# JosephCatrambone/aruco3

Measured on AMD Instinct MI355X. Metric: frames/sec at 1920x1080 ARUCO dict, higher is better.
Workload: dtype u8

## Files before the change

### aruco3_amd/csrc/k_contours.hip

```cpp
#include <algorithm>
#include <cmath>

#include "a3_common.h"
#include "a3_launch.h"


namespace a3 {

constexpr int kFinB = 8;
constexpr int kScatB = 1;

struct Nb8 { uint64_t c; uint64_t n[8]; };

__device__ __forceinline__ uint64_t ldw(const uint64_t* __restrict__ img, int wpr, int H, int j, int y) {
    return (y >= 0 && y < H && j >= 0 && j < wpr) ? img[(size_t)y * wpr + j] : 0ull;
}

__device__ __forceinline__ void pdart_words(const Nb8& nb, uint64_t p[8]) {
#pragma unroll
    for (int k = 0; k < 8; k++) {
        uint64_t m = nb.c & nb.n[k] & ~nb.n[(k + 7) & 7];
        if ((k & 1) == 0) m &= ~nb.n[(k + 6) & 7];
        p[k] = m;
    }
// ... 1055 lines not shown

__global__ __launch_bounds__(256) void k_resolve_eval(const FinState* __restrict__ fin, uint32_t n_darts, int W,
                                                      const uint64_t* __restrict__ d_rec, const uint64_t* __restrict__ t_cur,
                                                      uint64_t* __restrict__ t_next, int iter, DeviceCounters* __restrict__ ctr,
                                                      const uint32_t* __restrict__ n_live) {
    if (!ctr->resolve_needed || (iter > 0 && ctr->resolve_changed[iter - 1] == 0)) return;
    if (n_live) n_darts = min(n_darts, *n_live);
    for (uint32_t d = blockIdx.x * blockDim.x + threadIdx.x; d < n_darts; d += gridDim.x * blockDim.x) {
        const uint64_t rec = d_rec[d];
        const uint32_t info = rec_info(rec);
        if (!(info & (kInfoW | kInfoE))) continue;
        const uint32_t my_leader = fin[d].leader;
        if (fin[my_leader].leader != my_leader) { atomicOr(&ctr->err_flags, kErrBrokenEvent); continue; }
        const uint32_t xy = rec_xy(rec);
        const uint32_t x = xy & 0xFFFF, y = xy >> 16;
        const uint32_t q = y * (uint32_t)W + x;
        const uint32_t F = rec_F(rec), P = pdart_mask(F);
        const int k = info & 7;
        const uint32_t base = d - __popc(P & ((1u << k) - 1u));
        const int cnt = __popc(P);
        bool wfires = true;
        for (int i = 0; i < cnt; i++) {
            const uint32_t leader = fin[base + i].leader;
            const uint32_t t = (uint32_t)(t_cur[leader] >> 32);
            if (t < 2u * q) { wfires = false; break; }
        }
        const bool has_w = x > 0 && !(F & 1u);
        uint32_t key = kNoKey;
        if ((info & kInfoW) && wfires) key = 2u * q;
        else if ((info & kInfoE) && !(has_w && wfires)) key = 2u * q + 1u;
        if (key != kNoKey) atomicMin(reinterpret_cast<unsigned long long*>(&t_next[my_leader]),
                                     (unsigned long long)(((uint64_t)key << 32) | d));
    }
}

__global__ void k_resolve_commit(const FinState* __restrict__ fin, uint32_t n_darts, uint64_t* __restrict__ t_cur,
                                 uint64_t* __restrict__ t_next, int iter, int last, DeviceCounters* __restrict__ ctr,
                                 const uint32_t* __restrict__ n_live) {
    if (!ctr->resolve_needed || (iter > 0 && ctr->resolve_changed[iter - 1] == 0)) return;
    if (n_live) n_darts = min(n_darts, *n_live);
    uint32_t changed = 0;
    for (uint32_t d = blockIdx.x * blockDim.x + threadIdx.x; d < n_darts; d += gridDim.x * blockDim.x) {
        if (fin[d].leader != d) continue;
        const uint64_t a = t_cur[d], b = t_next[d];
        if (a != b) { changed++; t_cur[d] = b; }
        t_next[d] = kInf64;
    }
    for (int o = 32; o > 0; o >>= 1) changed += __shfl_down(changed, o);
    if ((threadIdx.x & 63) == 0 && changed) {
        atomicAdd(&ctr->resolve_changed[iter], changed);
        if (last) atomicOr(&ctr->err_flags, kErrResolve);
    }
}

__global__ __launch_bounds__(256) void k_cycle_select(FinState* fin, const uint32_t* __restrict__ leader_list,
                                                      const unsigned int* __restrict__ leader_count, const uint32_t* __restrict__ d_succ,
                                                      const uint64_t* __restrict__ t_cur, const uint32_t* __restrict__ frame_base,
                                                      uint32_t n_frames, uint32_t first_frame, uint32_t min_edge_length, double eps_factor,
                                                      double image_diag, ContourRec* __restrict__ contours,
                                                      uint32_t* __restrict__ cyc_start_off, uint32_t max_contours, uint64_t max_points,
                                                      DeviceCounters* __restrict__ ctr, uint32_t shard_cap, const uint64_t* __restrict__ d_rec,
                                                      int W ,
                                                      uint32_t* __restrict__ keep_tmp ,
                                                      int keep_all ,
                                                      const EntryState* __restrict__ es ) {
    if (ctr->entry_overflow) return;
    __shared__ uint32_t s_wave[4], s_wave_t[4];
    __shared__ unsigned long long s_wave_p[4];
    __shared__ uint32_t s_cbase;
    __shared__ unsigned long long s_pbase;
    const int lane = threadIdx.x & 63, wave = threadIdx.x >> 6;
    uint32_t n_max = 0;
    for (uint32_t sh = 0; sh < kLeaderShards; sh++) n_max = max(n_max, leader_count[sh]);
    const uint32_t span = (n_max + 63u) & ~63u;
    const uint32_t n_leaders = span * kLeaderShards;
    const uint32_t stride = gridDim.x * blockDim.x;

    struct Eval { bool valid, traced, keep, broken; uint32_t n, d; uint64_t t; };
    auto eval = [&](uint32_t i0) -> Eval {
        Eval e{false, false, false, false, 0u, 0u, kInf64};
        const uint32_t sh = i0 / span, i = i0 - sh * span;
        e.valid = i < leader_count[sh];
        if (!e.valid) return e;
        e.d = leader_list[(size_t)sh * shard_cap + i];
        e.t = W > 0 ? dart_key(e.d, d_rec[e.d], W) : t_cur[e.d];
        e.traced = e.t != kInf64;
        if (!e.traced) return e;
        const uint32_t sl = d_succ[e.d];
        const FinState fsl = fin_final(fin[sl], sl, es);
        if (sl == e.d || fsl.leader != e.d) { e.broken = true; return e; }
        e.n = (fsl.w & kFinHops) + 1u;
        const double eps = (double)e.n * eps_factor;
        e.keep = keep_all || (e.n >= 5u && (uint64_t)e.n * e.n >= 8ull * min_edge_length && eps < image_diag + 1.0);
        return e;
    };

    uint32_t my_keep = 0, my_traced = 0;
    unsigned long long my_points = 0;
    bool broken = false, moved = false;
    for (uint32_t i0 = blockIdx.x * blockDim.x + threadIdx.x; i0 < n_leaders; i0 += stride) {
        const Eval e = eval(i0);
        my_traced += e.traced; my_keep += e.keep; my_points += e.keep ? e.n : 0u;
        broken |= e.broken;
        if (e.valid) { const uint32_t sh = i0 / span; keep_tmp[(size_t)sh * shard_cap + (i0 - sh * span)] = e.keep ? 1u : 0u; }
        if (W > 0 && e.valid && !natural_start_fires(e.d, fin, es, d_rec, W)) moved = true;
    }
    if (moved) ctr->resolve_needed = 1u;
    if (broken) atomicOr(&ctr->err_flags, kErrBrokenEvent);
    uint32_t inc_k = my_keep, inc_t = my_traced;
    unsigned long long inc_p = my_points;
#define A3_DPP_ADD64(V, CTRL, RM)                                                                                       \
    {                                                                                                                    \
        const uint32_t lo_ = (uint32_t)__builtin_amdgcn_update_dpp(0, (int)(uint32_t)(V), CTRL, RM, 0xF, false);           \
        const uint32_t hi_ = (uint32_t)__builtin_amdgcn_update_dpp(0, (int)(uint32_t)((V) >> 32), CTRL, RM, 0xF, false);    \
        (V) += ((unsigned long long)hi_ << 32) | lo_;                                                                    \
    }
#define A3_DPP_ADD32(V, CTRL, RM) (V) += (uint32_t)__builtin_amdgcn_update_dpp(0, (int)(V), CTRL, RM, 0xF, false);
#define A3_STEP(CTRL, RM) A3_DPP_ADD32(inc_k, CTRL, RM) A3_DPP_ADD32(inc_t, CTRL, RM) A3_DPP_ADD64(inc_p, CTRL, RM)
    A3_STEP(0x111, 0xF) A3_STEP(0x112, 0xF) A3_STEP(0x114, 0xF) A3_STEP(0x118, 0xF) A3_STEP(0x142, 0xA) A3_STEP(0x143, 0xC)
#undef A3_STEP
#undef A3_DPP_ADD32
#undef A3_DPP_ADD64
    if (lane == 63) { s_wave[wave] = inc_k; s_wave_p[wave] = inc_p; s_wave_t[wave] = inc_t; }
    __syncthreads();
    uint32_t base_k = 0, tot_k = 0;
    unsigned long long base_p = 0, tot_p = 0;
    for (int w = 0; w < 4; w++) {
        if (w < wave) { base_k += s_wave[w]; base_p += s_wave_p[w]; }
        tot_k += s_wave[w]; tot_p += s_wave_p[w];
    }
    if (threadIdx.x == 0) {
        const uint32_t tot_t = s_wave_t[0] + s_wave_t[1] + s_wave_t[2] + s_wave_t[3];
        if (tot_t) atomicAdd(&ctr->traced, tot_t);
        s_cbase = tot_k ? atomicAdd(&ctr->contours, tot_k) : 0u;
        s_pbase = tot_k ? atomicAdd(&ctr->points, tot_p) : 0ull;
    }
    __syncthreads();
    uint32_t c = s_cbase + base_k + (inc_k - my_keep);
    unsigned long long pb = s_pbase + base_p + (inc_p - my_points);

    for (uint32_t i0 = blockIdx.x * blockDim.x + threadIdx.x; i0 < n_leaders; i0 += stride) {
        {
            const uint32_t sh = i0 / span, i = i0 - sh * span;
            if (i >= leader_count[sh]) continue;
            if (!keep_tmp[(size_t)sh * shard_cap + i]) { const uint32_t d = leader_list[(size_t)sh * shard_cap + i]; fin[d] = FinState{d, kFinEvent | kFinHops}; continue; }
        }
        const Eval e = eval(i0);
        if (!e.valid) continue;
        uint32_t slot = kNone;
        if (e.keep) {
            if (c >= max_contours || c >= kFinHops) atomicOr(&ctr->err_flags, kErrContourTable);
            else if (pb + e.n > max_points) atomicOr(&ctr->err_flags, kErrPointPool);
            else {
                uint32_t lo = 0, hi = n_frames;
                while (hi - lo > 1) { const uint32_t mid = (lo + hi) >> 1; if (frame_base[mid] <= e.d) lo = mid; else hi = mid; }
                ContourRec r;
                r.frame = first_frame + lo;
                r.start_key = (uint32_t)(e.t >> 32);
                r.point_base = (uint32_t)pb;
                r.n = e.n;
                contours[c] = r;
                cyc_start_off[c] = (uint32_t)e.t == e.d ? 0u : fin_final(fin[(uint32_t)e.t], (uint32_t)e.t, es).w & kFinHops;
                slot = c;
            }
            c++; pb += e.n;
        }
        fin[e.d] = FinState{e.d, kFinEvent | (slot == kNone ? kFinHops : slot)};
    }
}

__global__ __launch_bounds__(256) void k_scatter_points(const FinState* __restrict__ fin, uint32_t n_darts, const uint64_t* __restrict__ d_rec,
                                                        const ContourRec* __restrict__ contours,
                                                        const uint32_t* __restrict__ cyc_start_off, uint32_t* __restrict__ points,
                                                        const uint32_t* __restrict__ n_live, DeviceCounters* __restrict__ ctr,
                                                        uint32_t max_contours, uint64_t max_points,
                                                        const EntryState* __restrict__ es ) {
    if (ctr->entry_overflow) return;
    if (n_live) n_darts = min(n_darts, *n_live);
    const uint32_t n_contours = min(ctr->contours, max_contours);
    bool bad = false;
    constexpr int B = kScatB;
    const uint32_t stride = gridDim.x * blockDim.x;
    for (uint32_t d0 = blockIdx.x * blockDim.x + threadIdx.x; d0 < n_darts; d0 += B * stride) {
        FinState s[B];
        uint64_t rec[B];
        uint32_t c[B], so[B];
        FinState ls[B];
        ContourRec r[B];
        bool live[B];
#pragma unroll
        for (int u = 0; u < B; u++) {
            const uint32_t d = min(d0 + (uint32_t)u * stride, n_darts - 1u);
            s[u] = fin_final(fin[d], d, es);
        }
#pragma unroll
        for (int u = 0; u < B; u++) {
            live[u] = d0 + (uint32_t)u * stride < n_darts && (s[u].w & kFinEvent) != 0u &&
                      (s[u].w & kFinDead) == 0u;
            const uint32_t leader = live[u] ? s[u].leader : 0u;
            ls[u] = fin[leader];
            c[u] = ls[u].w & kFinHops;
            rec[u] = live[u] ? d_rec[min(d0 + (uint32_t)u * stride, n_darts - 1u)] : 0ull;
        }
#pragma unroll
        for (int u = 0; u < B; u++) {
            const bool named = live[u] && ls[u].leader == s[u].leader && c[u] != kFinHops;
            live[u] = named && c[u] < n_contours;
            bad |= named && !live[u];
            r[u] = contours[live[u] ? c[u] : 0u];
            so[u] = cyc_start_off[live[u] ? c[u] : 0u];
        }
#pragma unroll
        for (int u = 0; u < B; u++) {
            if (!live[u]) continue;
            const uint32_t off = s[u].leader == d0 + (uint32_t)u * stride ? 0u : s[u].w & kFinHops;
            const uint32_t rank = so[u] >= off ? so[u] - off : so[u] + r[u].n - off;
            if (rank < r[u].n && (uint64_t)r[u].point_base + rank < max_points) points[r[u].point_base + rank] = rec_xy(rec[u]);
            else bad = true;
        }
    }
    if (bad) atomicOr(&ctr->err_flags, kErrScatter);
}

__device__ __forceinline__ int orient(int px, int py, int qx, int qy, int rx, int ry) {
    const long long v = (long long)(qy - py) * (rx - qx) - (long long)(qx - px) * (ry - qy);
    return v == 0 ? 0 : (v > 0 ? 1 : -1);
}

__device__ bool hull4(const int* __restrict__ in , int* __restrict__ out ) {
    int sp = 0;
    for (int i = 1; i < 4; i++)
        if (in[2 * i + 1] < in[2 * sp + 1] || (in[2 * i + 1] == in[2 * sp + 1] && in[2 * i] < in[2 * sp])) sp = i;
    const int sx = in[2 * sp], sy = in[2 * sp + 1];
    int qx[3], qy[3];
    {
        int tx[4], ty[4];
        for (int i = 0; i < 4; i++) { tx[i] = in[2 * i]; ty[i] = in[2 * i + 1]; }
        tx[sp] = tx[0]; ty[sp] = ty[0];
        for (int i = 0; i < 3; i++) { qx[i] = tx[i + 1]; qy[i] = ty[i + 1]; }
    }
    for (int i = 1; i < 3; i++) {
        const int ax = qx[i], ay = qy[i];
        int j = i;
        while (j > 0) {
            const int bx = qx[j - 1], by = qy[j - 1];
            const int o = orient(sx, sy, ax, ay, bx, by);
            bool less;
            if (o == 0) {
                const long long da = (long long)(ax - sx) * (ax - sx) + (long long)(ay - sy) * (ay - sy);
                const long long db = (long long)(bx - sx) * (bx - sx) + (long long)(by - sy) * (by - sy);
                less = da < db;
            } else less = (o == -1);
            if (!less) break;
            qx[j] = bx; qy[j] = by; j--;
        }
        qx[j] = ax; qy[j] = ay;
    }
    int hx[5], hy[5], sn = 1;
    hx[0] = sx; hy[0] = sy;
    for (int i = 0; i < 3; i++) {
        while (sn > 1 && orient(hx[sn - 2], hy[sn - 2], hx[sn - 1], hy[sn - 1], qx[i], qy[i]) != -1) sn--;
        hx[sn] = qx[i]; hy[sn] = qy[i]; sn++;
    }
    if (sn != 4) return false;
    for (int i = 0; i < 4; i++) { out[2 * i] = hx[i]; out[2 * i + 1] = hy[i]; }
    return true;
}

__device__ __forceinline__ void enforce_clockwise(int* __restrict__ hq ) {
    const int dx1 = hq[2] - hq[0], dy1 = hq[3] - hq[1], dx2 = hq[4] - hq[0], dy2 = hq[5] - hq[1];
    if (dx1 * dy2 - dy1 * dx2 < 0) { const int tx = hq[2], ty = hq[3]; hq[2] = hq[6]; hq[3] = hq[7]; hq[6] = tx; hq[7] = ty; }
}

__global__ void k_debug_clockwise(const int32_t* __restrict__ in, uint32_t n, int32_t* __restrict__ out) {
    const uint32_t i = blockIdx.x * blockDim.x + threadIdx.x;
    if (i >= n) return;
    int q[8];
    for (int k = 0; k < 8; k++) q[k] = in[8 * i + k];
    enforce_clockwise(q);
    for (int k = 0; k < 8; k++) out[8 * i + k] = q[k];
}

#define A3_DPP_MAX64(V, CTRL, ROWMASK)                                                                                   \
    {                                                                                                                    \
        const uint32_t lo_ = (uint32_t)__builtin_amdgcn_update_dpp(0, (int)(uint32_t)(V), CTRL, ROWMASK, 0xF, false);        \
        const uint32_t hi_ = (uint32_t)__builtin_amdgcn_update_dpp(0, (int)(uint32_t)((V) >> 32), CTRL, ROWMASK, 0xF, false); \
        const unsigned long long o_ = ((unsigned long long)hi_ << 32) | lo_;                                             \
        (V) = o_ > (V) ? o_ : (V);                                                                                       \
    }
template <int G>
__device__ __forceinline__ unsigned long long group_max_u64(unsigned long long v) {
    A3_DPP_MAX64(v, 0x111, 0xF)
    A3_DPP_MAX64(v, 0x112, 0xF)
    A3_DPP_MAX64(v, 0x114, 0xF)
    A3_DPP_MAX64(v, 0x118, 0xF)
    if constexpr (G == 16) return __shfl(v, 15, 16);
    A3_DPP_MAX64(v, 0x142, 0xA)
    A3_DPP_MAX64(v, 0x143, 0xC)
    const uint32_t lo = (uint32_t)__builtin_amdgcn_readlane((int)(uint32_t)v, 63), hi = (uint32_t)__builtin_amdgcn_readlane((int)(uint32_t)(v >> 32), 63);
    return ((unsigned long long)hi << 32) | lo;
}
#undef A3_DPP_MAX64

constexpr uint32_t kSmallBorder = 64;
template <int G>
__device__ __forceinline__ void contour_quads_body(uint32_t block, uint32_t n_blocks, const ContourRec* __restrict__ contours, const DeviceCounters* __restrict__ ctr,
                                                       uint32_t max_contours, const uint32_t* __restrict__ points, double eps_factor,
                                                       uint32_t min_edge_length, uint32_t first_frame, uint32_t max_cand,
                                                       CandRec* __restrict__ cands, uint32_t* __restrict__ cand_count,
                                                       unsigned int* __restrict__ err_flags, bool coords14) {
    if (ctr->err_flags & (kErrPointPool | kErrContourTable)) return;
    const uint32_t n_contours = min(ctr->contours, max_contours);
    const int lane = threadIdx.x & (G - 1);
    const uint32_t wave_global = (block * blockDim.x + threadIdx.x) / G, n_waves = (n_blocks * blockDim.x) / G;
    for (uint32_t c = wave_global; c < n_contours; c += n_waves) {
        const ContourRec r = contours[c];
        if ((r.n <= kSmallBorder) != (G == 16)) continue;
        const uint32_t* P = points + r.point_base;
        const uint32_t n = r.n;
        const double eps = (double)n * eps_factor;
        uint32_t seg_a[8], seg_b[8];
        int nseg = 1, splits = 0;
        uint32_t kept[3];
        seg_a[0] = 0; seg_b[0] = n - 1;
        bool reject = false;
        while (nseg > 0 && !reject) {
            nseg--;
            const uint32_t a = seg_a[nseg], b = seg_b[nseg];
            const uint32_t pa = P[a], pb = P[b];
            const int ax = pa & 0xFFFF, ay = pa >> 16, bx = pb & 0xFFFF, by = pb >> 16;
            const int la = ay - by, lb = bx - ax;
            const long long lc = (long long)ax * by - (long long)bx * ay;
            unsigned long long best = 0;
            for (uint32_t i0 = a + 1 + lane; i0 <= b; i0 += 4 * G) {
                uint32_t p[4];
#pragma unroll
                for (int u = 0; u < 4; u++) p[u] = P[min(i0 + (uint32_t)u * G, b)];
#pragma unroll
                for (int u = 0; u < 4; u++) {
                    const uint32_t i = i0 + (uint32_t)u * G;
                    if (i > b) break;
                    unsigned long long anum;
                    if (coords14) {
                        const int v = __mul24(la, (int)(p[u] & 0xFFFF)) + __mul24(lb, (int)(p[u] >> 16)) + (int)lc;
                        anum = (unsigned long long)(uint32_t)(v < 0 ? -v : v);
                    } else {
                        long long num = (long long)la * (int)(p[u] & 0xFFFF) + (long long)lb * (int)(p[u] >> 16) + lc;
                        anum = (unsigned long long)(num < 0 ? -num : num);
                    }
                    const unsigned long long cand = (anum << 30) | (unsigned long long)(~i & 0x3FFFFFFFu);
                    if (cand > best) best = cand;
                }
            }
            best = group_max_u64<G>(best);
            const unsigned long long num = best >> 30;
            if (num == 0) continue;
            const uint32_t index = ~(uint32_t)best & 0x3FFFFFFFu;
            const double dn = (double)num, den = (double)((long long)la * la + (long long)lb * lb);
            const double lhs = dn * dn, rhs = eps * eps * den;
            bool far;
            if (lhs > rhs * (1.0 + 1e-9)) far = true;
            else if (lhs < rhs * (1.0 - 1e-9)) far = false;
            else far = dn / sqrt(den) > eps;
            if (far) {
                if (splits == 3) { reject = true; break; }
                kept[splits++] = index;
                seg_a[nseg] = a; seg_b[nseg] = index; nseg++;
                seg_a[nseg] = index; seg_b[nseg] = b; nseg++;
            }
        }
        if (reject || splits != 3) continue;
        if (lane != 0) continue;
        uint32_t k0 = kept[0], k1 = kept[1], k2 = kept[2], t;
        if (k0 > k1) { t = k0; k0 = k1; k1 = t; }
        if (k1 > k2) { t = k1; k1 = k2; k2 = t; }
        if (k0 > k1) { t = k0; k0 = k1; k1 = t; }
        const uint32_t idx[4] = {0u, k0, k1, k2};
        int q[8], hq[8];
        for (int i = 0; i < 4; i++) { const uint32_t p = P[idx[i]]; q[2 * i] = p & 0xFFFF; q[2 * i + 1] = p >> 16; }
        if (!hull4(q, hq)) continue;
        uint32_t cmin = min_edge_length + 1u;
        for (int i = 0; i < 4; i++) {
            const int j = (i + 1) & 3;
            const int dx = hq[2 * i] - hq[2 * j], dy = hq[2 * i + 1] - hq[2 * j + 1];
            const uint32_t d2 = (uint32_t)(dx * dx + dy * dy);
            cmin = d2 < cmin ? d2 : cmin;
        }
        if (cmin < min_edge_length) continue;
        enforce_clockwise(hq);
        const uint32_t fl = r.frame - first_frame;
        const uint32_t slot = atomicAdd(&cand_count[fl], 1u);
        if (slot >= max_cand) { atomicOr(err_flags, kErrCandTable); continue; }
        CandRec cr;
        cr.start_key = r.start_key;
        for (int i = 0; i < 8; i++) cr.xy[i] = (uint16_t)hq[i];
        cands[(size_t)fl * max_cand + slot] = cr;
    }
}

__global__ __launch_bounds__(256) void k_contour_quads(uint32_t blocks64, const ContourRec* __restrict__ contours, const DeviceCounters* __restrict__ ctr,
                                                       uint32_t max_contours, const uint32_t* __restrict__ points, double eps_factor,
                                                       uint32_t min_edge_length, uint32_t first_frame, uint32_t max_cand,
                                                       CandRec* __restrict__ cands, uint32_t* __restrict__ cand_count,
                                                       unsigned int* __restrict__ err_flags, int coords14) {
    if (blockIdx.x < blocks64)
        contour_quads_body<64>(blockIdx.x, blocks64, contours, ctr, max_contours, points, eps_factor, min_edge_length, first_frame, max_cand, cands,
                               cand_count, err_flags, coords14 != 0);
    else
        contour_quads_body<16>(blockIdx.x - blocks64, gridDim.x - blocks64, contours, ctr, max_contours, points, eps_factor, min_edge_length,
                               first_frame, max_cand, cands, cand_count, err_flags, coords14 != 0);
}

__global__ void k_unpack_bits(const uint64_t* __restrict__ bits, int W, int H, uint8_t* __restrict__ out) {
    const int x = blockIdx.x * blockDim.x + threadIdx.x, y = blockIdx.y;
    if (x >= W) return;
    const int wpr = (int)words_per_row((uint32_t)W);
    out[(size_t)y * W + x] = ((bits[(size_t)y * wpr + (x >> 6)] >> (x & 63)) & 1ull) ? 255 : 0;
}

constexpr int kFinBlocks = 1536;
static inline int blocks_for(uint64_t n, int per_block, int cap) {
    uint64_t b = (n + per_block - 1) / per_block;
    if (b < 1) b = 1;
    if (b > (uint64_t)cap) b = cap;
    return (int)b;
}

__global__ __launch_bounds__(256) void k_zero(uint4* __restrict__ p, uint32_t n16) {
    for (uint32_t i = blockIdx.x * blockDim.x + threadIdx.x; i < n16; i += gridDim.x * blockDim.x) p[i] = make_uint4(0u, 0u, 0u, 0u);
}
hipError_t launch_zero(hipStream_t st, void* p, size_t bytes) {
    const uint32_t n16 = (uint32_t)(bytes / 16);
    hipLaunchKernelGGL(k_zero, dim3(blocks_for(n16, 256, 256)), dim3(256), 0, st, reinterpret_cast<uint4*>(p), n16);
    return hipGetLastError();
}

static size_t tile_off_offset(uint32_t W, uint32_t H, uint32_t n_frames) { return (size_t)dart_tiles(W, H) * n_frames; }
static size_t tile_mask_offset_bytes(uint32_t W, uint32_t H, uint32_t n_frames) { return ((size_t)dart_tiles(W, H) * n_frames * 4 * (1 + kCountHalves) + 7) & ~(size_t)7; }
size_t tile_darts_bytes(uint32_t W, uint32_t H, uint32_t n_frames) { return tile_mask_offset_bytes(W, H, n_frames) + (size_t)dart_tiles(W, H) * n_frames * kCountHalves * 8; }

hipError_t launch_dart_count(hipStream_t st, const DartCountLaunch& d) {
    const uint64_t* const bits = d.bits; const int W = d.W, H = d.H; const uint32_t first_frame = d.first_frame, n_frames = d.n_frames;
    unsigned long long* const frame_darts = d.frame_darts; uint32_t* const tile_darts = d.tile_darts; PlanWords* const plan = d.plan;
    const uint32_t tiles_x = dart_tiles_x((uint32_t)W), tiles_y = ((uint32_t)H + kTileRows - 1) / kTileRows;
    const uint32_t wpr = words_per_row((uint32_t)W);
    uint32_t* h1 = tile_darts + (size_t)tiles_x * tiles_y * n_frames * 2;
    unsigned long long* tmask = reinterpret_cast<unsigned long long*>(reinterpret_cast<uint8_t*>(tile_darts) + tile_mask_offset_bytes((uint32_t)W, (uint32_t)H, n_frames));
    if (wpr <= 30)
        hipLaunchKernelGGL(k_dart_count<32>, dim3((tiles_y + 1) / 2, n_frames, kCountHalves), dim3(64), 0, st, bits, W, H, first_frame, frame_darts, tile_darts, h1, tmask);
    else
        hipLaunchKernelGGL(k_dart_count<64>, dim3(((wpr + kCountLanes - 1) / kCountLanes) * tiles_y, n_frames, kCountHalves), dim3(64), 0, st, bits, W, H, first_frame,
                           frame_darts, tile_darts, h1, tmask);
    hipLaunchKernelGGL(k_tile_scan, dim3(n_frames + (plan ? 1u : 0u)), dim3(256), 0, st, tile_darts, h1, tiles_x * tiles_y, first_frame,
                       tile_darts + (size_t)tiles_x * tiles_y * n_frames, n_frames, frame_darts, (unsigned long long)d.plan_cap, d.frame_base, plan,
                       reinterpret_cast<uint4*>(d.zero_p), (uint32_t)(d.zero_bytes / 16));
    return hipGetLastError();
}

hipError_t launch_dart_build(hipStream_t st, const ContourChunk& c) {
    const uint32_t tiles = dart_tiles((uint32_t)c.W, (uint32_t)c.H);
    const uint32_t* const tile_off = c.tile_darts + tile_off_offset((uint32_t)c.W, (uint32_t)c.H, c.batch_frames);
    const unsigned long long* const tile_mask = reinterpret_cast<const unsigned long long*>(
        reinterpret_cast<const uint8_t*>(c.tile_darts) + tile_mask_offset_bytes((uint32_t)c.W, (uint32_t)c.H, c.batch_frames));
    hipLaunchKernelGGL(k_dart_assign, dim3((tiles * c.n_frames + 7u) / 8u * 8u), dim3(256), 0, st, c.bits, c.W, c.H, c.first_frame, c.frame_base, tile_off,
                       c.pix_base, c.tile_darts, c.d_rec, c.d_succ, c.n_live, c.dbg, tile_mask, tiles, c.n_frames);
    if (c.dbg && c.dbg != 5) return hipGetLastError();
    hipLaunchKernelGGL(k_dart_link, dim3(blocks_for(c.n_darts, 256, 4096)), dim3(256), 0, st, c.W, c.H, c.first_frame, c.pix_base, c.bits, c.d_rec, c.d_succ,
                       c.n_darts, c.n_live);
    return hipGetLastError();
}

size_t entry_state_bytes() { return sizeof(EntryState); }
static bool finalize_inline(bool frame_entries, bool trust_natural) { return frame_entries && trust_natural; }
size_t fin_state_bytes() { return sizeof(FinState); }
size_t entry_slots(uint32_t n_darts) { return (size_t)entry_shard_cap(n_darts) * kEntryShards; }
size_t leader_list_bytes(uint32_t n_darts) { return (size_t)leader_shard_cap(n_darts) * kLeaderShards * 4; }

hipError_t launch_rank_cycles(hipStream_t st, const ContourChunk& c) {
    const uint32_t n_darts = c.n_darts, n_frames = c.n_frames, min_edge_length = c.min_edge_length; const int W = c.W, dbg = c.dbg, phase = c.phase;
    const uint64_t* const d_rec = c.d_rec; const uint32_t* const d_succ = c.d_succ, * const n_live = c.n_live, * const frame_base = c.frame_base;
    uint32_t* const entry_list = c.entry_list, * const leader_list = c.leader_list, * const frame_entries = c.frame_entries;
    unsigned int* const entry_count = c.entry_count, * const leader_count = c.leader_count, * const dead_count = c.dead_count;
    DeviceCounters* const ctr = c.ctr;
    const int trust_natural = c.inline_resolve_W > 0 ? 1 : 0;
    const uint32_t ecap = entry_shard_cap(n_darts);
    FinState* fin = reinterpret_cast<FinState*>(c.fin);
    const bool no_finalize = finalize_inline(frame_entries != nullptr, trust_natural != 0) && dbg == 0;
    uint32_t* const ll = no_finalize ? leader_list : nullptr;
    const uint32_t lcap = leader_shard_cap(n_darts);
    if (phase != 2) {
        if (frame_entries && !dead_count)
            hipLaunchKernelGGL((k_local_contract<kLTFrame, false>), dim3((n_darts + kLTFrame - 1) / kLTFrame), dim3(256), 0, st, n_darts, W, d_rec, d_succ, fin,
                               entry_list, entry_count, ecap, frame_base, frame_entries, n_live, dbg, min_edge_length, dead_count, trust_natural,
                               ll, leader_count, lcap);
        else if (frame_entries)
            hipLaunchKernelGGL((k_local_contract<kLTFrame, true>), dim3((n_darts + kLTFrame - 1) / kLTFrame), dim3(256), 0, st, n_darts, W, d_rec, d_succ, fin,
                               entry_list, entry_count, ecap, frame_base, frame_entries, n_live, dbg, min_edge_length, dead_count, trust_natural,
                               ll, leader_count, lcap);
        else
            hipLaunchKernelGGL((k_local_contract<kLT, true>), dim3((n_darts + kLT - 1) / kLT), dim3(256), 0, st, n_darts, W, d_rec, d_succ, fin,
                               entry_list, entry_count, ecap, frame_base, frame_entries, n_live, dbg, min_edge_length, dead_count, trust_natural,
                               ll, leader_count, lcap);
    }
    if (dbg || phase == 1) return hipGetLastError();
    EntryState* a = reinterpret_cast<EntryState*>(c.es_a);
    EntryState* b = reinterpret_cast<EntryState*>(c.es_b);
    if (frame_entries) {
        hipLaunchKernelGGL(k_entry_frame, dim3(n_frames), dim3(256), 0, st, entry_list, frame_entries, frame_base, fin, d_rec, W, a, ctr,
                           ll, leader_count, lcap);
        if (no_finalize) return hipGetLastError();
        const int fin_blocks = std::max(blocks_for(n_darts, 256, kFinBlocks), (int)(((uint64_t)n_darts + 256ull * 32 - 1) / (256ull * 32)));
        hipLaunchKernelGGL(k_jump_finalize, dim3(fin_blocks), dim3(256), 0, st, n_darts, a, fin,
                           leader_list, leader_count, leader_shard_cap(n_darts), n_live, ctr);
        return hipGetLastError();
    }
    const dim3 grid(blocks_for(n_darts / 16 + 1, 256, 1024)), block(256);
    hipLaunchKernelGGL(k_entry_init, grid, block, 0, st, entry_list, entry_count, fin, d_rec, W, a, ecap);
    for (int r = 0; r < c.max_rounds; r++) {
        hipLaunchKernelGGL(k_entry_jump, grid, block, 0, st, a, b, entry_count, ecap, r, ctr);
        EntryState* t = a; a = b; b = t;
    }
    const int fin_blocks = std::max(blocks_for(n_darts, 256, kFinBlocks), (int)(((uint64_t)n_darts + 256ull * 32 - 1) / (256ull * 32)));
    hipLaunchKernelGGL(k_jump_finalize, dim3(fin_blocks), block, 0, st, n_darts, a, fin,
                       leader_list, leader_count, leader_shard_cap(n_darts), n_live, ctr);
    return hipGetLastError();
}

hipError_t launch_resolve(hipStream_t st, const ContourChunk& c) {
    const uint32_t n_darts = c.n_darts; const int W = c.W, max_iters = c.resolve_iters;
    const uint64_t* const d_rec = c.d_rec; uint64_t* const t_cur = c.t_cur, * const t_next = c.t_next;
    const uint32_t* const leader_list = c.leader_list, * const n_live = c.n_live; const unsigned int* const leader_count = c.leader_count;
    DeviceCounters* const ctr = c.ctr;
    const FinState* fin = reinterpret_cast<const FinState*>(c.fin);
    if (max_iters <= 0) return hipSuccess;
    const dim3 grid(blocks_for(n_darts, 256, 4096)), block(256);
    hipLaunchKernelGGL(k_resolve_fast, dim3(blocks_for(n_darts / 16 + 1, 256, 1024)), block, 0, st, fin, leader_list, leader_count,
                       leader_shard_cap(n_darts), W, d_rec, t_cur, ctr);
    hipLaunchKernelGGL(k_resolve_init, grid, block, 0, st, fin, d_rec, W, n_darts, t_cur, t_next, ctr, n_live);
    for (int it = 0; it < max_iters; it++) {
        hipLaunchKernelGGL(k_resolve_eval, grid, block, 0, st, fin, n_darts, W, d_rec, t_cur, t_next, it, ctr, n_live);
        hipLaunchKernelGGL(k_resolve_commit, grid, block, 0, st, fin, n_darts, t_cur, t_next, it, it == max_iters - 1 ? 1 : 0, ctr, n_live);
    }
    return hipGetLastError();
}

hipError_t launch_select_scatter(hipStream_t st, const ContourChunk& c) {
    const uint32_t n_darts = c.n_darts;
    const double image_diag = std::sqrt((double)c.W * c.W + (double)c.H * c.H);
    const EntryState* es = finalize_inline(c.frame_entries != nullptr, c.inline_resolve_W > 0) ? reinterpret_cast<const EntryState*>(c.es_a) : nullptr;
    const dim3 grid(blocks_for(n_darts, 256, (int)std::min<uint32_t>(65536u, std::max<uint32_t>(8192u, n_darts / 1024u)))), block(256);
    hipLaunchKernelGGL(k_cycle_select, dim3(blocks_for(n_darts / 64 + 1, 256, 1024)), block, 0, st, reinterpret_cast<FinState*>(c.fin), c.leader_list, c.leader_count,
                       c.d_succ, c.t_cur, c.frame_base, c.n_frames, c.first_frame, c.min_edge_length,
                       c.eps_factor, image_diag, c.contours, c.cyc_start_off, c.max_contours, c.max_points, c.ctr, leader_shard_cap(n_darts), c.d_rec,
                       c.inline_resolve_W, c.leader_keep, c.keep_all ? 1 : 0, es);
    hipLaunchKernelGGL(k_scatter_points, grid, block, 0, st, reinterpret_cast<const FinState*>(c.fin), n_darts, c.d_rec, c.contours, c.cyc_start_off, c.points, c.n_live,
                       c.ctr, c.max_contours, c.max_points, es);
    return hipGetLastError();
}

hipError_t launch_contour_quads(hipStream_t st, const ContourChunk& c) {
    const uint32_t n_darts = c.n_darts;
    const int coords14 = c.W <= 16384 && c.H <= 16384 ? 1 : 0;
    const uint32_t b64 = std::min<uint32_t>(2560u, std::max<uint32_t>(40u, n_darts / 2048u)),
                   b16 = std::min<uint32_t>(4096u, std::max<uint32_t>(64u, n_darts / 1024u));
    hipLaunchKernelGGL(k_contour_quads, dim3(b64 + b16), dim3(256), 0, st, b64, c.contours, c.ctr,
                       c.max_contours, c.points, c.eps_factor, c.min_edge_length, c.first_frame, c.max_cand,
                       c.cands + (size_t)c.first_frame * c.max_cand, c.cand_count + c.first_frame, c.err_flags, coords14);
    return hipGetLastError();
}

hipError_t launch_debug_clockwise(hipStream_t st, const int32_t* in, uint32_t n, int32_t* out) {
    hipLaunchKernelGGL(k_debug_clockwise, dim3((n + 63) / 64), dim3(64), 0, st, in, n, out);
    return hipGetLastError();
}

hipError_t launch_unpack_bits(hipStream_t st, const uint64_t* bits, int W, int H, uint8_t* out) {
    hipLaunchKernelGGL(k_unpack_bits, dim3((W + 255) / 256, H), dim3(256), 0, st, bits, W, H, out);
    return hipGetLastError();
}

}
```

Baseline: 376,400.

## Keep contour points register-resident during Douglas-Peucker quad fitting

For contours that fit in G*R lanes-by-rows, points are loaded once into registers as packed keys and every Douglas-Peucker split scans those registers instead of re-reading global memory. The argmax uses 32-bit DPP max/min reductions in place of the 64-bit packed reduction, and a register-based segment stack replaces the small local arrays. Kept vertex coordinates are carried along so the final hull step needs no reload, and a waves_per_eu(6) hint is added. The trade is higher register pressure from holding up to 16 keys per lane, which may reduce occupancy.

New measurement: 381,300 (median of 5 runs). No clear change (+1.3%).

```diff
diff --git a/aruco3_amd/csrc/k_contours.hip b/aruco3_amd/csrc/k_contours.hip
--- a/aruco3_amd/csrc/k_contours.hip
+++ b/aruco3_amd/csrc/k_contours.hip
@@ -1381,7 +1381,107 @@
 }
 #undef A3_DPP_MAX64
 
+#define A3_DPP_RED32(V, OP, IDENT, CTRL, ROWMASK) \
+    (V) = OP((V), (uint32_t)__builtin_amdgcn_update_dpp((int)(IDENT), (int)(V), CTRL, ROWMASK, 0xF, false));
+#define A3_GROUP_RED32(NAME, OP, IDENT)                                                             \
+    template <int G>                                                                                \
+    __device__ __forceinline__ uint32_t NAME(uint32_t v) {                                          \
+        if constexpr (G == 16) {                                                                    \
+            A3_DPP_RED32(v, OP, IDENT, 0x121, 0xF)                         \
+            A3_DPP_RED32(v, OP, IDENT, 0x122, 0xF)                                                  \
+            A3_DPP_RED32(v, OP, IDENT, 0x124, 0xF)                                                  \
+            A3_DPP_RED32(v, OP, IDENT, 0x128, 0xF)                                                  \
+            return v;                                                                               \
+        } else {                                                                                    \
+            A3_DPP_RED32(v, OP, IDENT, 0x111, 0xF)                         \
+            A3_DPP_RED32(v, OP, IDENT, 0x112, 0xF)                                                  \
+            A3_DPP_RED32(v, OP, IDENT, 0x114, 0xF)                                                  \
+            A3_DPP_RED32(v, OP, IDENT, 0x118, 0xF)                                                  \
+            A3_DPP_RED32(v, OP, IDENT, 0x142, 0xA)              \
+            A3_DPP_RED32(v, OP, IDENT, 0x143, 0xC)              \
+            return (uint32_t)__builtin_amdgcn_readlane((int)v, 63);                                 \
+        }                                                                                           \
+    }
+A3_GROUP_RED32(group_max_u32, max, 0u)
+A3_GROUP_RED32(group_min_u32, min, 0xFFFFFFFFu)
+#undef A3_GROUP_RED32
+#undef A3_DPP_RED32
+
+template <int G>
+__device__ __forceinline__ uint32_t group_read(uint32_t v, uint32_t src) {
+    if constexpr (G == 16) return (uint32_t)__shfl((int)v, (int)src, 16);
+    else return (uint32_t)__builtin_amdgcn_readlane((int)v, (int)src);
+}
+
 constexpr uint32_t kSmallBorder = 64;
+
+struct ChordEnds {
+    uint32_t e0, e1, e2, e3, e4;
+    __device__ __forceinline__ void pop(uint32_t& a, uint32_t& b) { a = e1; b = e0; e0 = e1; e1 = e2; e2 = e3; e3 = e4; }
+    __device__ __forceinline__ void split(uint32_t mid, uint32_t b) { e4 = e2; e3 = e1; e2 = e0; e1 = mid; e0 = b; }
+};
+
+constexpr int kResidentRows64 = 16, kResidentRows16 = (int)kSmallBorder / 16;
+__device__ __forceinline__ uint32_t resident_key(uint32_t p, int row) { return (p & 0xFFFFu) << 18 | (uint32_t)row << 14 | p >> 16; }
+__device__ __forceinline__ uint32_t resident_point(uint32_t key) { return key >> 18 | (key & 0x3FFFu) << 16; }
+template <int G, int R>
+__device__ __forceinline__ bool dp_resident(const uint32_t* __restrict__ P, uint32_t n, double eps, int lane, uint32_t (&kept)[3],
+                                            uint32_t (&kept_pt)[3], uint32_t& p0) {
+    static_assert(R <= 16, "the row has four bits");
+    uint32_t key[R];
+#pragma unroll
+    for (int u = 0; u < R; u++) {
+        key[u] = P[min((uint32_t)(u * G + lane), n - 1u)];
+    }
+    const uint32_t first = P[0], last = P[n - 1];
+#pragma unroll
+    for (int u = 0; u < R; u++) key[u] = resident_key(key[u], u);
+    p0 = first;
+    ChordEnds at{n - 1, 0, 0, 0, 0}, pt{resident_key(last, 0), resident_key(first, 0), 0, 0, 0};
+    int nseg = 1, splits = 0;
+    while (nseg > 0) {
+        nseg--;
+        uint32_t a, b, pa, pb;
+        at.pop(a, b);
+        pt.pop(pa, pb);
+        if (a == b) continue;
+        const int ax = pa >> 18, ay = pa & 0x3FFF, bx = pb >> 18, by = pb & 0x3FFF;
+        const int la = ay - by, lb = bx - ax, lc = ax * by - bx * ay;
+        uint32_t best_num = 0, best_key = 0;
+        const uint32_t off = (uint32_t)lane - (a + 1u), span = b - a;
+        const uint32_t u_lo = (a + 1u) / G, u_span = b / G - u_lo;
+        uint32_t x_shift = 18u, y_mask = 0x3FFFu;
+        asm volatile("" : "+s"(x_shift), "+s"(y_mask));
+#pragma unroll
+        for (int u = 0; u < R; u++) {
+            if constexpr (G == 64)
+                if ((uint32_t)u - u_lo > u_span) continue;
+            const int v = __mul24(la, (int)(key[u] >> x_shift)) + __mul24(lb, (int)(key[u] & y_mask)) + lc;
+            uint32_t num = (uint32_t)(v < 0 ? -v : v);
+            num = off + (uint32_t)(u * G) < span ? num : 0u;
+            if (num > best_num) { best_num = num; best_key = key[u]; }
+        }
+        const uint32_t num = group_max_u32<G>(best_num);
+        if (num == 0) continue;
+        const uint32_t index = group_min_u32<G>(best_num == num ? (best_key >> 14 & 15u) * (uint32_t)G + (uint32_t)lane : 0xFFFFFFFFu);
+        const uint32_t pi = group_read<G>(best_key, index & (uint32_t)(G - 1));
+        const double dn = (double)num, den = (double)((long long)la * la + (long long)lb * lb);
+        const double lhs = dn * dn, rhs = eps * eps * den;
+        bool far;
+        if (lhs > rhs * (1.0 + 1e-9)) far = true;
+        else if (lhs < rhs * (1.0 - 1e-9)) far = false;
+        else far = dn / sqrt(den) > eps;
+        if (far) {
+            if (splits == 3) return false;
+            kept[splits] = index; kept_pt[splits] = resident_point(pi); splits++;
+            at.split(index, b);
+            pt.split(pi, pb);
+            nseg += 2;
+        }
+    }
+    return splits == 3;
+}
+
 template <int G>
 __device__ __forceinline__ void contour_quads_body(uint32_t block, uint32_t n_blocks, const ContourRec* __restrict__ contours, const DeviceCounters* __restrict__ ctr,
                                                        uint32_t max_contours, const uint32_t* __restrict__ points, double eps_factor,
@@ -1391,72 +1491,82 @@
     if (ctr->err_flags & (kErrPointPool | kErrContourTable)) return;
     const uint32_t n_contours = min(ctr->contours, max_contours);
     const int lane = threadIdx.x & (G - 1);
-    const uint32_t wave_global = (block * blockDim.x + threadIdx.x) / G, n_waves = (n_blocks * blockDim.x) / G;
+    uint32_t wave_global = (block * blockDim.x + threadIdx.x) / G;
+    const uint32_t n_waves = (n_blocks * blockDim.x) / G;
+    if constexpr (G == 64) wave_global = (uint32_t)__builtin_amdgcn_readfirstlane((int)wave_global);
+    constexpr int R = G == 64 ? kResidentRows64 : kResidentRows16;
     for (uint32_t c = wave_global; c < n_contours; c += n_waves) {
         const ContourRec r = contours[c];
         if ((r.n <= kSmallBorder) != (G == 16)) continue;
         const uint32_t* P = points + r.point_base;
         const uint32_t n = r.n;
         const double eps = (double)n * eps_factor;
-        uint32_t seg_a[8], seg_b[8];
-        int nseg = 1, splits = 0;
-        uint32_t kept[3];
-        seg_a[0] = 0; seg_b[0] = n - 1;
-        bool reject = false;
-        while (nseg > 0 && !reject) {
-            nseg--;
-            const uint32_t a = seg_a[nseg], b = seg_b[nseg];
-            const uint32_t pa = P[a], pb = P[b];
-            const int ax = pa & 0xFFFF, ay = pa >> 16, bx = pb & 0xFFFF, by = pb >> 16;
-            const int la = ay - by, lb = bx - ax;
-            const long long lc = (long long)ax * by - (long long)bx * ay;
-            unsigned long long best = 0;
-            for (uint32_t i0 = a + 1 + lane; i0 <= b; i0 += 4 * G) {
-                uint32_t p[4];
-#pragma unroll
-                for (int u = 0; u < 4; u++) p[u] = P[min(i0 + (uint32_t)u * G, b)];
-#pragma unroll
-                for (int u = 0; u < 4; u++) {
-                    const uint32_t i = i0 + (uint32_t)u * G;
-                    if (i > b) break;
-                    unsigned long long anum;
-                    if (coords14) {
-                        const int v = __mul24(la, (int)(p[u] & 0xFFFF)) + __mul24(lb, (int)(p[u] >> 16)) + (int)lc;
-                        anum = (unsigned long long)(uint32_t)(v < 0 ? -v : v);
-                    } else {
-                        long long num = (long long)la * (int)(p[u] & 0xFFFF) + (long long)lb * (int)(p[u] >> 16) + lc;
-                        anum = (unsigned long long)(num < 0 ? -num : num);
+        uint32_t kept[3], kept_pt[3] = {0u, 0u, 0u}, p0 = 0;
+        const bool resident = coords14 && n <= (uint32_t)(G * R);
+        if (resident) {
+            if (!dp_resident<G, R>(P, n, eps, lane, kept, kept_pt, p0)) continue;
+        } else {
+            ChordEnds at{n - 1, 0, 0, 0, 0};
+            int nseg = 1, splits = 0;
+            bool reject = false;
+            while (nseg > 0 && !reject) {
+                nseg--;
+                uint32_t a, b;
+                at.pop(a, b);
+                const uint32_t pa = P[a], pb = P[b];
+                const int ax = pa & 0xFFFF, ay = pa >> 16, bx = pb & 0xFFFF, by = pb >> 16;
+                const int la = ay - by, lb = bx - ax;
+                const long long lc = (long long)ax * by - (long long)bx * ay;
+                unsigned long long best = 0;
+                for (uint32_t i0 = a + 1 + lane; i0 <= b; i0 += 4 * G) {
+                    uint32_t p[4];
+#pragma unroll
+                    for (int u = 0; u < 4; u++) p[u] = P[min(i0 + (uint32_t)u * G, b)];
+#pragma unroll
+                    for (int u = 0; u < 4; u++) {
+                        const uint32_t i = i0 + (uint32_t)u * G;
+                        if (i > b) break;
+                        unsigned long long anum;
+                        if (coords14) {
+                            const int v = __mul24(la, (int)(p[u] & 0xFFFF)) + __mul24(lb, (int)(p[u] >> 16)) + (int)lc;
+                            anum = (unsigned long long)(uint32_t)(v < 0 ? -v : v);
+                        } else {
+                            long long num = (long long)la * (int)(p[u] & 0xFFFF) + (long long)lb * (int)(p[u] >> 16) + lc;
+                            anum = (unsigned long long)(num < 0 ? -num : num);
+                        }
+                        const unsigned long long cand = (anum << 30) | (unsigned long long)(~i & 0x3FFFFFFFu);
+                        if (cand > best) best = cand;
                     }
-                    const unsigned long long cand = (anum << 30) | (unsigned long long)(~i & 0x3FFFFFFFu);
-                    if (cand > best) best = cand;
+                }
+                best = group_max_u64<G>(best);
+                const unsigned long long num = best >> 30;
+                if (num == 0) continue;
+                const uint32_t index = ~(uint32_t)best & 0x3FFFFFFFu;
+                const double dn = (double)num, den = (double)((long long)la * la + (long long)lb * lb);
+                const double lhs = dn * dn, rhs = eps * eps * den;
+                bool far;
+                if (lhs > rhs * (1.0 + 1e-9)) far = true;
+                else if (lhs < rhs * (1.0 - 1e-9)) far = false;
+                else far = dn / sqrt(den) > eps;
+                if (far) {
+                    if (splits == 3) { reject = true; break; }
+                    kept[splits++] = index;
+                    at.split(index, b);
+                    nseg += 2;
                 }
             }
-            best = group_max_u64<G>(best);
-            const unsigned long long num = best >> 30;
-            if (num == 0) continue;
-            const uint32_t index = ~(uint32_t)best & 0x3FFFFFFFu;
-            const double dn = (double)num, den = (double)((long long)la * la + (long long)lb * lb);
-            const double lhs = dn * dn, rhs = eps * eps * den;
-            bool far;
-            if (lhs > rhs * (1.0 + 1e-9)) far = true;
-            else if (lhs < rhs * (1.0 - 1e-9)) far = false;
-            else far = dn / sqrt(den) > eps;
-            if (far) {
-                if (splits == 3) { reject = true; break; }
-                kept[splits++] = index;
-                seg_a[nseg] = a; seg_b[nseg] = index; nseg++;
-                seg_a[nseg] = index; seg_b[nseg] = b; nseg++;
-            }
-        }
-        if (reject || splits != 3) continue;
+            if (reject || splits != 3) continue;
+        }
         if (lane != 0) continue;
         uint32_t k0 = kept[0], k1 = kept[1], k2 = kept[2], t;
-        if (k0 > k1) { t = k0; k0 = k1; k1 = t; }
-        if (k1 > k2) { t = k1; k1 = k2; k2 = t; }
-        if (k0 > k1) { t = k0; k0 = k1; k1 = t; }
+        uint32_t q0 = kept_pt[0], q1 = kept_pt[1], q2 = kept_pt[2];
+        if (k0 > k1) { t = k0; k0 = k1; k1 = t; t = q0; q0 = q1; q1 = t; }
+        if (k1 > k2) { t = k1; k1 = k2; k2 = t; t = q1; q1 = q2; q2 = t; }
+        if (k0 > k1) { t = k0; k0 = k1; k1 = t; t = q0; q0 = q1; q1 = t; }
         const uint32_t idx[4] = {0u, k0, k1, k2};
+        const uint32_t pts[4] = {p0, q0, q1, q2};
         int q[8], hq[8];
-        for (int i = 0; i < 4; i++) { const uint32_t p = P[idx[i]]; q[2 * i] = p & 0xFFFF; q[2 * i + 1] = p >> 16; }
+        for (int i = 0; i < 4; i++) { const uint32_t p = resident ? pts[i] : P[idx[i]]; q[2 * i] = p & 0xFFFF; q[2 * i + 1] = p >> 16; }
         if (!hull4(q, hq)) continue;
         uint32_t cmin = min_edge_length + 1u;
         for (int i = 0; i < 4; i++) {
@@ -1477,7 +1587,7 @@
     }
 }
 
-__global__ __launch_bounds__(256) void k_contour_quads(uint32_t blocks64, const ContourRec* __restrict__ contours, const DeviceCounters* __restrict__ ctr,
+__global__ __launch_bounds__(256) __attribute__((amdgpu_waves_per_eu(6))) void k_contour_quads(uint32_t blocks64, const ContourRec* __restrict__ contours, const DeviceCounters* __restrict__ ctr,
                                                        uint32_t max_contours, const uint32_t* __restrict__ points, double eps_factor,
                                                        uint32_t min_edge_length, uint32_t first_frame, uint32_t max_cand,
                                                        CandRec* __restrict__ cands, uint32_t* __restrict__ cand_count,
```
